# olegroshka/vae-channel-dynamics

Measured on AMD Instinct MI355X. Metric: images/sec SDXL-VAE train step @256x256 (tracking on), higher is better.
Workload: dtype f32

## Files before the change

### vae-channel-dynamics_amd/csrc/igemm.hip

```cpp
#include "bf16_frag.h"
#include <algorithm>
#include <stdlib.h>
#include <type_traits>

#include "launchers.h"

namespace {

struct LanePos {
  int lr, lh, trq, trp, trh;
};
__device__ __forceinline__ LanePos lane_pos(int lane) { return LanePos{lane & 31, lane >> 5, (lane & 15) >> 2, lane & 3, (lane >> 4) & 1}; }

struct F32 {
  typedef float elem;
  typedef f32x4 raw4;
  typedef f32x4 frag;
  typedef unsigned off_t;
  static constexpr int BK_ROWS = 32, BK_WGRAD = 32;
  static constexpr int KG = 8;
  static constexpr int PAD_K = 4, PAD_T = 4;
  static constexpr bool SETPRIO = true;
  static constexpr bool PAIR16 = false;
  static constexpr bool flag(int32_t) { return false; }

  static __device__ __forceinline__ raw4 load4(__amdgpu_buffer_rsrc_t rs, unsigned, bool ok, int row, int ld, int c) {
    return VAE_BUF_LOAD4(rs, oob_unless(ok, ((unsigned)row * (unsigned)ld + (unsigned)c) * 4u));
  }
  static __device__ __forceinline__ f32x4 to_f32(raw4 r, bool) { return r; }
  static __device__ __forceinline__ void put4(elem* d, f32x4 v) { *reinterpret_cast<f32x4*>(d) = v; }
  static __device__ __forceinline__ void put4_stored(elem* d, raw4, f32x4 v, bool) { put4(d, v); }
  static __device__ __forceinline__ frag frag_k(const elem* p) { return *reinterpret_cast<const f32x4*>(p); }
  static __device__ __forceinline__ frag frag_t(const elem* tile, int ld, int kg, LanePos l, int col0) {
    frag v;
#pragma unroll
    for (int j = 0; j < 4; ++j) v[j] = tile[(kg * 8 + l.lh * 4 + j) * ld + col0 + l.lr];
    return v;
  }
  template <int MI, int NI>
  static __device__ __forceinline__ void frags_tt(frag* a, frag* b, const elem* sA, int ldA, int colA, const elem* sB, int ldB, int colB, int kg, LanePos l) {
#pragma unroll
    for (int j = 0; j < 4; ++j) {
      const int k = kg * 8 + l.lh * 4 + j;
#pragma unroll
      for (int mi = 0; mi < MI; ++mi) a[mi][j] = sA[k * ldA + colA + mi * 32 + l.lr];
#pragma unroll
      for (int ni = 0; ni < NI; ++ni) b[ni][j] = sB[k * ldB + colB + ni * 32 + l.lr];
    }
  }
  template <int MI, int NI>
  static __device__ __forceinline__ void mma(f32x16 (&acc)[MI][NI], const frag* a, const frag* b) {
#pragma unroll
    for (int j = 0; j < 4; ++j)
#pragma unroll
      for (int mi = 0; mi < MI; ++mi)
#pragma unroll
        for (int ni = 0; ni < NI; ++ni) acc[mi][ni] = __builtin_amdgcn_mfma_f32_32x32x2f32(a[mi][j], b[ni][j], acc[mi][ni], 0, 0, 0);
  }
  static __device__ __forceinline__ off_t out_off(bool ok, int orow, int ldc, int col) {
    return ok ? ((unsigned)orow * (unsigned)ldc + (unsigned)col) * 4u : BUF_OOB;
  }
  static __device__ __forceinline__ bool inside(off_t o) { return o != BUF_OOB; }
  static __device__ __forceinline__ float load1(__amdgpu_buffer_rsrc_t rs, bool, off_t o) {
    return __builtin_bit_cast(float, __builtin_amdgcn_raw_buffer_load_b32(rs, o, 0, 0));
  }
  static __device__ __forceinline__ void store1(__amdgpu_buffer_rsrc_t rs, bool, off_t o, float v) {
    __builtin_amdgcn_raw_buffer_store_b32(__builtin_bit_cast(unsigned, v), rs, o, 0, 0);
  }
};

struct BF16 {
  typedef u16 elem;
  typedef uint4 raw4;
  typedef bf16x8 frag;
  typedef int off_t;
  static constexpr int BK_ROWS = 64, BK_WGRAD = 32;
  static constexpr int KG = 16;
  static constexpr int PAD_K = 8, PAD_T = 32;
  static constexpr bool SETPRIO = false;
  static constexpr bool PAIR16 = true;
  static __device__ __forceinline__ bool flag(int32_t v) { return v != 0; }

  static __device__ __forceinline__ raw4 load4(__amdgpu_buffer_rsrc_t rs, unsigned esize, bool ok, int row, int ld, int c) {
    return buf_load4_raw(rs, esize, neg_unless(ok, row * ld + c));
  }
  static __device__ __forceinline__ f32x4 to_f32(raw4 r, bool bf) { return raw4_to_f32(r, bf); }
  static __device__ __forceinline__ void put4(elem* d, f32x4 v) { *reinterpret_cast<uint2*>(d) = pack4(v); }
  static __device__ __forceinline__ void put4_stored(elem* d, raw4 r, f32x4 v, bool bf) {
    *reinterpret_cast<uint2*>(d) = bf ? uint2{r.x, r.y} : pack4(v);
  }
  static __device__ __forceinline__ frag frag_k(const elem* p) { return frag_direct(p); }
  static __device__ __forceinline__ frag frag_t(const elem* tile, int ld, int kg, LanePos l, int col0) {
    return frag_tr(tile + (kg * 16 + l.lh * 8 + l.trq) * ld + col0 + l.trh * 16 + l.trp * 4, ld);
  }
  template <int MI, int NI>
  static __device__ __forceinline__ void frags_tt(frag* a, frag* b, const elem* sA, int ldA, int colA, const elem* sB, int ldB, int colB, int kg, LanePos l) {
#pragma unroll
    for (int mi = 0; mi < MI; ++mi) a[mi] = frag_t(sA, ldA, kg, l, colA + mi * 32);
#pragma unroll
    for (int ni = 0; ni < NI; ++ni) b[ni] = frag_t(sB, ldB, kg, l, colB + ni * 32);
  }
  template <int MI, int NI>
  static __device__ __forceinline__ void mma(f32x16 (&acc)[MI][NI], const frag* a, const frag* b) {
#pragma unroll
    for (int mi = 0; mi < MI; ++mi)
#pragma unroll
      for (int ni = 0; ni < NI; ++ni) acc[mi][ni] = __builtin_amdgcn_mfma_f32_32x32x16_bf16(a[mi], b[ni], acc[mi][ni], 0, 0, 0);
  }
  static __device__ __forceinline__ off_t out_off(bool ok, int orow, int ldc, int col) { return ok ? orow * ldc + col : -1; }
  static __device__ __forceinline__ bool inside(off_t o) { return o >= 0; }
  static __device__ __forceinline__ float load1(__amdgpu_buffer_rsrc_t rs, bool bf, off_t o) { return buf_load1_elem(rs, bf, o); }
  static __device__ __forceinline__ void store1(__amdgpu_buffer_rsrc_t rs, bool bf, off_t o, float v) { buf_store1_elem(rs, bf, o, v); }

  static __device__ __forceinline__ bool pair16(const vae_igemm_args& p, bool cbf, bool rbf, const char* C) {
    return cbf && (p.N % 2 == 0) && (p.ldc % 2 == 0) && (p.res == nullptr || rbf) && p.track == nullptr && ((reinterpret_cast<uintptr_t>(C) & 3u) == 0);
  }
  template <int MI, int NI, class RowPixel>
  static __device__ __forceinline__ void store_pairs(const vae_igemm_args& p, const f32x16 (&acc)[MI][NI], int ni, __amdgpu_buffer_rsrc_t rsC,
                                                     __amdgpu_buffer_rsrc_t rsR, int col, bool colok, int m0, int trow0, int lh, bool s2c,
                                                     RowPixel row_pixel) {
    const bool odd = col & 1;
    const float b0 = (p.bias && colok) ? p.bias[col & ~1] : 0.f, b1 = (p.bias && colok) ? p.bias[col | 1] : 0.f;
#pragma unroll
    for (int mi = 0; mi < MI; ++mi) {
      unsigned o16[8], rr[8];
#pragma unroll
      for (int j = 0; j < 8; ++j) {
        const int r = 2 * j + (odd ? 1 : 0);
        const int row = trow0 + mi * 32 + (r & 3) + 8 * (r >> 2) + 4 * lh;
        int orow = row;
        if (s2c) {
          int b, y, x;
          row_pixel(row < p.M ? row : m0, b, y, x);
          orow = (b * p.g.Ho + y) * p.g.Wo + x;
        }
        o16[j] = (colok && row < p.M) ? (unsigned)(orow * p.ldc + (col & ~1)) * 2u : BUF_OOB;
        rr[j] = 0u;
      }
      if (p.res) {
#pragma unroll
        for (int j = 0; j < 8; ++j) rr[j] = __builtin_amdgcn_raw_buffer_load_b32(rsR, o16[j], 0, 0);
      }
#pragma unroll
      for (int j = 0; j < 8; ++j) {
        const float a0 = p.alpha * acc[mi][ni][2 * j], a1 = p.alpha * acc[mi][ni][2 * j + 1];
        const float recv = lane_xor1(odd ? a0 : a1);
        typedef __bf16 bf16x2_t __attribute__((ext_vector_type(2)));
        bf16x2_t h;
        h[0] = (__bf16)((odd ? recv : a0) + b0 + __builtin_bit_cast(float, rr[j] << 16));
        h[1] = (__bf16)((odd ? a1 : recv) + b1 + __builtin_bit_cast(float, rr[j] & 0xffff0000u));
        __builtin_amdgcn_raw_buffer_store_b32(__builtin_bit_cast(unsigned, h), rsC, o16[j], 0, 0);
      }
    }
  }
};

template <int MI, int NI>
__device__ __forceinline__ void zero_acc(f32x16 (&acc)[MI][NI]) {
#pragma unroll
  for (int mi = 0; mi < MI; ++mi)
#pragma unroll
    for (int ni = 0; ni < NI; ++ni)
#pragma unroll
      for (int r = 0; r < 16; ++r) acc[mi][ni][r] = 0.f;
}

template <class P, int BM, int BN, int WM, int WN, bool BKM, bool VEC, int XF>
__device__ __forceinline__ void rows_body(const vae_igemm_args& p) {
  typedef typename P::elem elem;
  constexpr int BK = P::BK_ROWS;
  constexpr int NT = 64 * WM * WN;
  constexpr int KQ = BK / 4;
  constexpr int RP = NT / KQ;
  constexpr int LDA = BK + P::PAD_K;
  constexpr int LDB = BKM ? (BN + P::PAD_T) : (BK + P::PAD_K);
  constexpr int SA = BM * LDA;
  constexpr int SB = BKM ? BK * LDB : BN * LDB;
  constexpr int STAGE = SA + SB;
  constexpr int SS = (XF != VAE_XF_NONE) ? 2 * SS_HALF * (4 / (int)sizeof(elem)) : 0;
  constexpr int TM = BM / WM, TN = BN / WN, MI = TM / 32, NI = TN / 32;
  constexpr int AR = BM / RP;
  constexpr int NQ = BN / 4, KR = NT / NQ;
  constexpr int BR = BKM ? (BK / KR) : (BN / RP);
  static_assert(AR >= 1 && BR >= 1 && TM % 32 == 0 && TN % 32 == 0 && (BK / P::KG == 2 || BK / P::KG == 4), "tile/wave layout");
  __shared__ __attribute__((aligned(16))) elem smem[2 * STAGE + SS];
  float* sS = reinterpret_cast<float*>(smem + 2 * STAGE);

  const int tid = threadIdx.x, lane = tid & 63, wave = tid >> 6;
  const int wm = wave / WN, wn = wave % WN;
  const LanePos lp = lane_pos(lane);
  const int lr = lp.lr, lh = lp.lh;
  const int tilesN = (p.N + BN - 1) / BN;
  const int tm = blockIdx.x / tilesN, tn = blockIdx.x % tilesN;
  const int m0 = tm * BM, n0 = tn * BN;
  const int z = blockIdx.z;
  const vae_conv_geom g = p.g;
  const SrcMap smap = make_srcmap(g);
  const bool abf = P::flag(p.a_bf16), cbf = P::flag(p.out_bf16), rbf = P::flag(p.res_bf16);
  const unsigned esA = abf ? 2u : 4u;
  const char* __restrict__ A = reinterpret_cast<const char*>(p.A) + (int64_t)z * p.sAb * esA;
  const float* __restrict__ W = p.W + (int64_t)z * p.sWb;
  const int hw = g.Ho * g.Wo;

  const bool s2c = (g.mode == VAE_MODE_DGRAD_S2);
  const int hh = g.Ho >> 1, wh = g.Wo >> 1;
  const int cls_rows = s2c ? p.M >> 2 : 1;
  const int cls = s2c ? m0 / cls_rows : 0;
  const int cpy = cls >> 1, cpx = cls & 1;
  const int nkw = s2c ? (cpx ? 1 : 2) : 3;
  const int ntaps = s2c ? (cpy ? 1 : 2) * nkw : g.taps;
  auto row_pixel = [&](int m, int& b, int& y, int& x) {
    if (s2c) {
      const int r = m - cls * cls_rows;
      b = r / (hh * wh);
      const int rem = r - b * (hh * wh);
      const int i = rem / wh;
      y = 2 * i + cpy;
      x = 2 * (rem - i * wh) + cpx;
    } else {
      b = m / hw;
      const int rem = m - b * hw;
      y = rem / g.Wo;
      x = rem - y * g.Wo;
    }
  };

  const int b_base = s2c ? (m0 - cls * cls_rows) / (hh * wh) : m0 / hw;
  const size_t img = (size_t)g.Hs * g.Ws * g.Cs;
  const size_t abytes = (size_t)(g.B - b_base) * img * esA, wbytes = (size_t)(BKM ? (int64_t)p.K * p.sk : (int64_t)p.N * p.sn) * 4u;
  const auto rsA = VAE_BUF_RSRC(A + (int64_t)b_base * img * esA, abytes < BUF_MAX ? abytes : BUF_MAX);
  const auto rsW = VAE_BUF_RSRC(W, wbytes < BUF_MAX ? wbytes : BUF_MAX);

  const int k4 = tid % KQ, r0 = tid / KQ;
  const int n4 = tid % NQ, kq = tid / NQ;
  int rb[AR], ry[AR], rx[AR];
#pragma unroll
  for (int i = 0; i < AR; ++i) {
    const int m = m0 + r0 + RP * i;
// ... 26 lines not shown
  int a_b[AR];
  int reg_c0 = 0;

  auto load_regs = [&](int s) {
    const int ord = s / kchunks;
    const int c0 = (s - ord * kchunks) * BK;
    reg_c0 = c0;
    int kh, kw;
    if (s2c) {
      const int a = ord / nkw;
      kh = cpy ? 1 : 2 * a;
      kw = cpx ? 1 : 2 * (ord - a * nkw);
    } else {
      kh = (g.taps == 9) ? ord / 3 : 0;
      kw = (g.taps == 9) ? ord - kh * 3 : 0;
    }
    const int tap = kh * 3 + kw;
    const int c = c0 + k4 * 4;
#pragma unroll
    for (int i = 0; i < AR; ++i) {
      int sy = 0, sx = 0;
      const bool ok = src_pixel(smap, ry[i], rx[i], kh, kw, sy, sx) && (rb[i] >= 0);
      if constexpr (VEC) ra[i] = P::load4(rsA, esA, ok && c < p.K, ((rb[i] - b_base) * g.Hs + sy) * g.Ws + sx, g.Cs, c);
      else ra[i] = load4s(p.A + (int64_t)z * p.sAb + (((int64_t)rb[i] * g.Hs + sy) * g.Ws + sx) * g.Cs + c, ok, c, p.K);
      a_b[i] = ok ? rb[i] : -1;
    }
    if (!BKM) {
#pragma unroll
      for (int i = 0; i < BR; ++i) {
        const int n = n0 + r0 + RP * i;
        if constexpr (VEC) rw[i] = VAE_BUF_LOAD4(rsW, oob_unless(n < p.N && c < p.K, ((unsigned)n * (unsigned)p.sn + (unsigned)tap * (unsigned)p.st + (unsigned)c) * 4u));
        else rw[i] = load4s(W + (int64_t)n * p.sn + (int64_t)tap * p.st + c, n < p.N, c, p.K);
      }
    } else {
#pragma unroll
      for (int i = 0; i < BR; ++i) {
        const int k = c0 + kq + KR * i;
        const int n = n0 + n4 * 4;
        if constexpr (VEC) rw[i] = VAE_BUF_LOAD4(rsW, oob_unless(k < p.K && n < p.N, ((unsigned)k * (unsigned)p.sk + (unsigned)tap * (unsigned)p.st + (unsigned)n) * 4u));
        else rw[i] = load4s(W + (int64_t)k * p.sk + (int64_t)tap * p.st + n, k < p.K, n, p.N);
      }
    }
  };
  auto store_lds = [&](elem* sA, elem* sB) {
    const int c = reg_c0 + k4 * 4;
#pragma unroll
    for (int i = 0; i < AR; ++i) {
      f32x4 v = P::to_f32(ra[i], abf);
      if (XF != VAE_XF_NONE) {
        const bool ok = (a_b[i] >= 0) && (c < p.K);
        const int o = ok ? (a_b[i] - b_lo) * p.K + c : 0;
        v = xform4_tab<XF>(v, sS + o, sS + SS_HALF + o, ok);
      }
      P::put4(&sA[(r0 + RP * i) * LDA + k4 * 4], v);
    }
#pragma unroll
    for (int i = 0; i < BR; ++i) {
      if (!BKM) P::put4(&sB[(r0 + RP * i) * LDB + k4 * 4], rw[i]);
      else P::put4(&sB[(kq + KR * i) * LDB + n4 * 4], rw[i]);
    }
  };
  typename P::frag fa[2][MI], fb[2][NI];
  auto fetch = [&](const elem* sA, const elem* sB, int kg, typename P::frag* a, typename P::frag* b) {
#pragma unroll
    for (int mi = 0; mi < MI; ++mi) a[mi] = P::frag_k(&sA[(wm * TM + mi * 32 + lr) * LDA + kg * P::KG + lh * (P::KG / 2)]);
#pragma unroll
    for (int ni = 0; ni < NI; ++ni) {
      if (!BKM) b[ni] = P::frag_k(&sB[(wn * TN + ni * 32 + lr) * LDB + kg * P::KG + lh * (P::KG / 2)]);
      else b[ni] = P::frag_t(sB, LDB, kg, lp, wn * TN + ni * 32);
    }
  };
  constexpr int NKG = BK / P::KG;
  auto compute = [&](const elem* sA, const elem* sB, int kg) {
    if (kg + 1 < NKG) fetch(sA, sB, kg + 1, fa[(kg + 1) & 1], fb[(kg + 1) & 1]);
    __builtin_amdgcn_sched_barrier(0);
    if (P::SETPRIO) __builtin_amdgcn_s_setprio(1);
    P::mma(acc, fa[kg & 1], fb[kg & 1]);
    if (P::SETPRIO) __builtin_amdgcn_s_setprio(0);
    __builtin_amdgcn_sched_barrier(0);
  };
  load_regs(0);
  __syncthreads();
  store_lds(smem, smem + SA);
  if (steps > 1) load_regs(1);
  __syncthreads();
  for (int s = 0; s < steps; ++s) {
    const elem* cA = smem + (s & 1) * STAGE;
    const elem* cB = cA + SA;
    fetch(cA, cB, 0, fa[0], fb[0]);
    compute(cA, cB, 0);
    if (NKG == 4) compute(cA, cB, 1);
    if (s + 1 < steps) {
      elem* nA = smem + ((s + 1) & 1) * STAGE;
      store_lds(nA, nA + SA);
      if (s + 2 < steps) load_regs(s + 2);
    }
    compute(cA, cB, NKG / 2);
    if (NKG == 4) compute(cA, cB, 3);
    __syncthreads();
  }

  const unsigned esC = cbf ? 2u : 4u, esR = rbf ? 2u : 4u;
  char* __restrict__ C = reinterpret_cast<char*>(p.C) + (int64_t)z * p.sCb * esC;
  const auto rsC = VAE_BUF_RSRC(C, (size_t)p.M * p.ldc * esC);
  const auto rsR = VAE_BUF_RSRC(p.res ? reinterpret_cast<const char*>(p.res) + (int64_t)z * p.sCb * esR : C, (size_t)p.M * p.ldc * (p.res ? esR : esC));
  float tsum[NI];
#pragma unroll
  for (int ni = 0; ni < NI; ++ni) tsum[ni] = 0.f;
  bool pair16 = false;
  if constexpr (P::PAIR16) pair16 = P::pair16(p, cbf, rbf, C);
#pragma unroll
  for (int ni = 0; ni < NI; ++ni) {
    const int col = n0 + wn * TN + ni * 32 + lr;
    const bool colok = col < p.N;
    const float bv = (p.bias && colok) ? p.bias[col] : 0.f;
    if constexpr (P::PAIR16) {
      if (pair16) {
        P::store_pairs(p, acc, ni, rsC, rsR, col, colok, m0, m0 + wm * TM, lh, s2c, row_pixel);
        continue;
      }
    }
#pragma unroll
    for (int mi = 0; mi < MI; ++mi) {
      typename P::off_t off[16];
      float rv[16];
#pragma unroll
      for (int r = 0; r < 16; ++r) {
        const int row = m0 + wm * TM + mi * 32 + (r & 3) + 8 * (r >> 2) + 4 * lh;
        int orow = row;
        if (s2c) {
          int b, y, x;
          row_pixel(row < p.M ? row : m0, b, y, x);
          orow = (b * g.Ho + y) * g.Wo + x;
        }
        off[r] = P::out_off(colok && row < p.M, orow, p.ldc, col);
        rv[r] = 0.f;
      }
      if (p.res) {
#pragma unroll
        for (int r = 0; r < 16; ++r) rv[r] = P::load1(rsR, rbf, off[r]);
      }
#pragma unroll
      for (int r = 0; r < 16; ++r) {
        const float v = p.alpha * acc[mi][ni][r] + bv + rv[r];
        P::store1(rsC, cbf, off[r], v);
        tsum[ni] += P::inside(off[r]) ? fabsf(v) : 0.f;
      }
    }
  }
  if (p.track && z == 0) {
    float* red = reinterpret_cast<float*>(smem);
#pragma unroll
    for (int ni = 0; ni < NI; ++ni) {
      const float s2 = tsum[ni] + __shfl_xor(tsum[ni], 32, 64);
      if (lh == 0) red[wm * BN + wn * TN + ni * 32 + lr] = s2;
    }
    __syncthreads();
    if (tid < BN) {
      float t = 0.f;
#pragma unroll
      for (int w = 0; w < WM; ++w) t += red[w * BN + tid];
      if (n0 + tid < p.N) p.track[(int64_t)tm * p.N + n0 + tid] = t;
    }
  }
}

template <class P, int BM, int BN, int WM, int WN, bool VEC, int XF>
__device__ __forceinline__ void wgrad_body(const vae_wgrad_args& p) {
  typedef typename P::elem elem;
  constexpr int BK = P::BK_WGRAD;
  constexpr int NT = 64 * WM * WN;
  constexpr int LDA = BM + P::PAD_T, LDB = BN + P::PAD_T;
  constexpr int SA = BK * LDA, SB = BK * LDB;
  constexpr int STAGE = SA + SB;
  constexpr int SS = (XF != VAE_XF_NONE) ? 2 * SS_HALF * (4 / (int)sizeof(elem)) : 0;
  constexpr int TM = BM / WM, TN = BN / WN, MI = TM / 32, NI = TN / 32;
  constexpr int AQ = BM / 4, AKR = NT / AQ, AI = BK / AKR;
  constexpr int BQ = BN / 4, BKR = NT / BQ, BI = BK / BKR;
  static_assert(AI >= 1 && BI >= 1 && TM % 32 == 0 && TN % 32 == 0 && (BK / P::KG == 2 || BK / P::KG == 4), "tile/wave layout");
  __shared__ __attribute__((aligned(16))) elem smem[2 * STAGE + SS];
  float* sS = reinterpret_cast<float*>(smem + 2 * STAGE);

  const int tid = threadIdx.x, lane = tid & 63, wave = tid >> 6;
  const int wm = wave / WN, wn = wave % WN;
  const LanePos lp = lane_pos(lane);
  const int lr = lp.lr, lh = lp.lh;
  const int tilesN = (p.N + BN - 1) / BN;
  const int tm = blockIdx.x / tilesN, tn = blockIdx.x % tilesN;
  const int m0 = tm * BM, n0 = tn * BN;
  const int tap = blockIdx.y / p.nsplit, split = blockIdx.y % p.nsplit;
  const int z = blockIdx.z;
  const vae_conv_geom g = p.g;
  const SrcMap smap = make_srcmap(g);
  const int kh = (g.taps == 9) ? tap / 3 : 0, kw = (g.taps == 9) ? tap - kh * 3 : 0;
  const bool ybf = P::flag(p.y_bf16), xbf = P::flag(p.x_bf16);
  const unsigned esY = ybf ? 2u : 4u, esX = xbf ? 2u : 4u;
  const char* __restrict__ dY = reinterpret_cast<const char*>(p.dY) + (int64_t)z * p.sYb * esY;
  const char* __restrict__ X = reinterpret_cast<const char*>(p.X) + (int64_t)z * p.sXb * esX;

  int chunk = (p.npix + p.nsplit - 1) / p.nsplit;
  chunk = ((chunk + 31) / 32) * 32;
  const int pbeg = split * chunk;
  const int pend = min(p.npix, pbeg + chunk);
  const int steps = (pend > pbeg) ? (pend - pbeg + BK - 1) / BK : 0;
  const int hw = g.Ho * g.Wo;
  const bool do_bias = (p.bias_partial != nullptr) && tn == 0 && tap == 0 && z == 0;

  const int b_lo = pbeg / hw;
  if (XF != VAE_XF_NONE && steps > 0) {
    const int nb = (pend - 1) / hw - b_lo + 1;
    const int ncol = min(BN, p.N - n0);
    const int nent = min(nb * BN, SS_HALF);
    for (int i = tid; i < nent; i += NT) {
      const int j = i / BN, c = i - j * BN;
      const bool ok = c < ncol;
      sS[i] = ok ? p.scale[(int64_t)(b_lo + j) * g.Cs + n0 + c] : 0.f;
      sS[SS_HALF + i] = ok ? p.shift[(int64_t)(b_lo + j) * g.Cs + n0 + c] : 0.f;
    }
  }

  f32x16 acc[MI][NI];
  zero_acc(acc);

  const size_t img = (size_t)g.Hs * g.Ws * g.Cs;
  const size_t ybytes = (size_t)(steps > 0 ? pend - pbeg : 0) * p.ldy * esY, xbytes = (size_t)(g.B - b_lo) * img * esX;
  const auto rsY = VAE_BUF_RSRC(dY + (int64_t)pbeg * p.ldy * esY, ybytes < BUF_MAX ? ybytes : BUF_MAX);
  const auto rsX = VAE_BUF_RSRC(X + (int64_t)b_lo * img * esX, xbytes < BUF_MAX ? xbytes : BUF_MAX);

  const int a4 = tid % AQ, akq = tid / AQ;
  const int b4 = tid % BQ, bkq = tid / BQ;
  typename P::raw4 ra[AI], rx[BI];
  int xb[BI];
  f32x4 bsum = {0.f, 0.f, 0.f, 0.f};

  auto load_regs = [&](int s) {
    const int pb = pbeg + s * BK;
#pragma unroll
    for (int i = 0; i < AI; ++i) {
      const int pix = pb + akq + AKR * i;
      const int c = m0 + a4 * 4;
      if constexpr (VEC) ra[i] = P::load4(rsY, esY, pix < pend && c < p.M, pix - pbeg, p.ldy, c);
      else ra[i] = load4s(p.dY + (int64_t)z * p.sYb + (int64_t)pix * p.ldy + c, pix < pend, c, p.M);
    }
#pragma unroll
    for (int i = 0; i < BI; ++i) {
      const int pix = pb + bkq + BKR * i;
      const int c = n0 + b4 * 4;
      const int b = pix / hw, rem = pix - b * hw;
      const int y = rem / g.Wo, x = rem - y * g.Wo;
      int sy = 0, sx = 0;
      const bool ok = src_pixel(smap, y, x, kh, kw, sy, sx) && (pix < pend);
      if constexpr (VEC) rx[i] = P::load4(rsX, esX, ok && c < p.N, ((b - b_lo) * g.Hs + sy) * g.Ws + sx, g.Cs, c);
      else rx[i] = load4s(p.X + (int64_t)z * p.sXb + (((int64_t)b * g.Hs + sy) * g.Ws + sx) * g.Cs + c, ok, c, p.N);
      xb[i] = ok ? b : -1;
    }
  };
  auto store_lds = [&](elem* sA, elem* sB) {
#pragma unroll
    for (int i = 0; i < AI; ++i) {
      const f32x4 v = P::to_f32(ra[i], ybf);
      P::put4_stored(&sA[(akq + AKR * i) * LDA + a4 * 4], ra[i], v, ybf);
      if (do_bias) bsum += v;
    }
#pragma unroll
    for (int i = 0; i < BI; ++i) {
      f32x4 v = P::to_f32(rx[i], xbf);
      if (XF != VAE_XF_NONE) {
        const bool ok = xb[i] >= 0;
        const int o = ok ? (xb[i] - b_lo) * BN + b4 * 4 : 0;
        v = xform4_tab<XF>(v, sS + o, sS + SS_HALF + o, ok);
      }
      P::put4(&sB[(bkq + BKR * i) * LDB + b4 * 4], v);
    }
  };
  typename P::frag fa[2][MI], fb[2][NI];
  auto fetch = [&](const elem* sA, const elem* sB, int kg, typename P::frag* a, typename P::frag* b) {
    P::template frags_tt<MI, NI>(a, b, sA, LDA, wm * TM, sB, LDB, wn * TN, kg, lp);
  };
  constexpr int NKG = BK / P::KG;
  auto compute = [&](const elem* sA, const elem* sB, int kg) {
    if (kg + 1 < NKG) fetch(sA, sB, kg + 1, fa[(kg + 1) & 1], fb[(kg + 1) & 1]);
    __builtin_amdgcn_sched_barrier(0);
    if (P::SETPRIO) __builtin_amdgcn_s_setprio(1);
    P::mma(acc, fa[kg & 1], fb[kg & 1]);
    if (P::SETPRIO) __builtin_amdgcn_s_setprio(0);
    __builtin_amdgcn_sched_barrier(0);
  };
  if (steps > 0) {
    load_regs(0);
    __syncthreads();
    store_lds(smem, smem + SA);
    if (steps > 1) load_regs(1);
    __syncthreads();
    for (int s = 0; s < steps; ++s) {
      const elem* cA = smem + (s & 1) * STAGE;
      const elem* cB = cA + SA;
      fetch(cA, cB, 0, fa[0], fb[0]);
      compute(cA, cB, 0);
      if (NKG == 4) compute(cA, cB, 1);
      if (s + 1 < steps) {
        elem* nA = smem + ((s + 1) & 1) * STAGE;
        store_lds(nA, nA + SA);
        if (s + 2 < steps) load_regs(s + 2);
      }
      compute(cA, cB, NKG / 2);
      if (NKG == 4) compute(cA, cB, 3);
      __syncthreads();
    }
  }

  const int64_t ld = (int64_t)g.taps * p.N;
  float* __restrict__ O = (p.nsplit == 1 ? p.out : p.partial + (int64_t)split * p.M * ld) + (int64_t)z * p.sOb;
#pragma unroll
  for (int ni = 0; ni < NI; ++ni) {
    const int col = n0 + wn * TN + ni * 32 + lr;
    if (col >= p.N) continue;
#pragma unroll
    for (int mi = 0; mi < MI; ++mi)
#pragma unroll
      for (int r = 0; r < 16; ++r) {
        const int row = m0 + wm * TM + mi * 32 + (r & 3) + 8 * (r >> 2) + 4 * lh;
        if (row < p.M) O[(int64_t)row * ld + (int64_t)tap * p.N + col] = p.alpha * acc[mi][ni][r];
      }
  }
  if (do_bias) {
    f32x4* red = reinterpret_cast<f32x4*>(smem);
    red[akq * AQ + a4] = bsum;
    __syncthreads();
    if (tid < AQ) {
      f32x4 t = {0.f, 0.f, 0.f, 0.f};
      for (int r = 0; r < AKR; ++r) t += red[r * AQ + tid];
#pragma unroll
      for (int e = 0; e < 4; ++e) {
        const int m = m0 + tid * 4 + e;
        if (m < p.M) p.bias_partial[(int64_t)split * p.M + m] = t[e];
      }
    }
  }
}

template <int BM, int BN, int WM, int WN, bool BKM, bool VEC, int XF>
__global__ __launch_bounds__(64 * WM * WN) void igemm_rows_kernel(vae_igemm_args p) { rows_body<F32, BM, BN, WM, WN, BKM, VEC, XF>(p); }
template <int BM, int BN, int WM, int WN, bool VEC, int XF>
__global__ __launch_bounds__(64 * WM * WN) void wgrad_kernel(vae_wgrad_args p) { wgrad_body<F32, BM, BN, WM, WN, VEC, XF>(p); }
template <int BM, int BN, int WM, int WN, bool BKM, int XF>
__global__ __launch_bounds__(64 * WM * WN) void igemm_rows_bf16_kernel(vae_igemm_args p) { rows_body<BF16, BM, BN, WM, WN, BKM, true, XF>(p); }
template <int BM, int BN, int WM, int WN, int XF>
__global__ __launch_bounds__(64 * WM * WN) void wgrad_bf16_kernel(vae_wgrad_args p) { wgrad_body<BF16, BM, BN, WM, WN, true, XF>(p); }

__device__ __forceinline__ void small_column_sums(const float* __restrict__ partial2, int nsplit, int n2, float* __restrict__ out2, int blk) {
  const int i = blk * 256 + (int)threadIdx.x;
  if (i >= n2) return;
  const float* p = partial2 + i;
  float s = 0.f;
  int k = 0;
  for (; k + 16 <= nsplit; k += 16) {
    float v[16];
#pragma unroll
    for (int j = 0; j < 16; ++j) v[j] = p[(int64_t)(k + j) * n2];
#pragma unroll
    for (int j = 0; j < 16; ++j) s += v[j];
  }
  for (; k < nsplit; ++k) s += p[(int64_t)k * n2];
  out2[i] = s;
}

template <int KP>
__global__ __launch_bounds__(256) void reduce_splits_kernel(const float* __restrict__ partial, int nsplit, int64_t n, float* __restrict__ out,
                                                            int main_blocks, const float* __restrict__ partial2, int n2, float* __restrict__ out2) {
  constexpr int COLS = 256 / KP;
  __shared__ f32x4 red[KP > 1 ? 256 : 1];
  if ((int)blockIdx.x >= main_blocks) {
    small_column_sums(partial2, nsplit, n2, out2, (int)blockIdx.x - main_blocks);
    return;
  }
  const int col = threadIdx.x % COLS, kp = threadIdx.x / COLS;
  const int64_t n4 = n >> 2;
  const int per = (nsplit + KP - 1) / KP;
  const int k0 = kp * per, k1 = min(nsplit, k0 + per);
  auto column = [&](int64_t i) {
    f32x4 s = {0.f, 0.f, 0.f, 0.f};
    const f32x4* p = reinterpret_cast<const f32x4*>(partial) + i;
    int k = k0;
    for (; k + 8 <= k1; k += 8) {
      f32x4 v[8];
#pragma unroll
      for (int j = 0; j < 8; ++j) v[j] = p[(int64_t)(k + j) * n4];
      s += ((v[0] + v[1]) + (v[2] + v[3])) + ((v[4] + v[5]) + (v[6] + v[7]));
    }
    for (; k < k1; ++k) s += p[(int64_t)k * n4];
    return s;
  };
  if (KP == 1) {
    for (int64_t i = (int64_t)blockIdx.x * 256 + threadIdx.x; i < n4; i += (int64_t)main_blocks * 256) reinterpret_cast<f32x4*>(out)[i] = column(i);
    return;
  }
  const int64_t i = (int64_t)blockIdx.x * COLS + col;
// ... 101 lines not shown
    f32x4 o[9];
    if constexpr (NPOS == 16) {
      f32x4 h[3][4];
#pragma unroll
      for (int j = 0; j < 4; ++j) {
        const float cj = (j == 1 || j == 2) ? 0.5f : 1.f;
        const f32x4 r0 = acc[0 * 4 + j] * cj, r1 = acc[1 * 4 + j] * (0.5f * cj), r2 = acc[2 * 4 + j] * (0.5f * cj), r3 = acc[3 * 4 + j] * cj;
        h[0][j] = (r0 + r1) + r2;
        h[1][j] = r1 - r2;
        h[2][j] = (r1 + r2) - r3;
      }
#pragma unroll
      for (int a = 0; a < 3; ++a) {
        o[a * 3 + 0] = (h[a][0] + h[a][1]) + h[a][2];
        o[a * 3 + 1] = h[a][1] - h[a][2];
        o[a * 3 + 2] = (h[a][1] + h[a][2]) - h[a][3];
      }
    } else {
      f32x4 h[3][3];
#pragma unroll
      for (int j = 0; j < 3; ++j) {
        h[0][j] = acc[0 * 3 + j] + acc[1 * 3 + j];
        h[1][j] = acc[1 * 3 + j];
        h[2][j] = acc[1 * 3 + j] - acc[2 * 3 + j];
      }
#pragma unroll
      for (int a = 0; a < 3; ++a) {
        o[a * 3 + 0] = h[a][0] + h[a][1];
        o[a * 3 + 1] = h[a][1];
        o[a * 3 + 2] = h[a][1] - h[a][2];
      }
    }
#pragma unroll
    for (int t = 0; t < 9; ++t)
#pragma unroll
      for (int e = 0; e < 4; ++e) sT[t][4 * cq + e][cl] = o[t][e];
  }
  __syncthreads();
  for (int idx = tid; idx < 9 * TCO * TCI; idx += 256) {
    const int c = idx % TCI, r = idx / TCI;
    const int t = r % 9, ml = r / 9;
    dW[((int64_t)(m0 + ml) * 9 + t) * N + c0 + c] = sT[t][ml][c];
  }
}

using std::false_type;
using std::true_type;

template <bool BF, int BM, int BN, int WM, int WN>
int launch_rows_tile(const vae_igemm_args& a, bool bkm, bool vec, hipStream_t st) {
  const dim3 grid((unsigned)(((a.M + BM - 1) / BM) * ((a.N + BN - 1) / BN)), 1, (unsigned)a.batch), block(64 * WM * WN);
  auto go = [&](auto bkm_c, auto vec_c) {
    constexpr bool BKM = decltype(bkm_c)::value, VEC = decltype(vec_c)::value;
    auto launch = [&](auto xf) {
      if constexpr (BF) hipLaunchKernelGGL((igemm_rows_bf16_kernel<BM, BN, WM, WN, BKM, decltype(xf)::value>), grid, block, 0, st, a);
      else hipLaunchKernelGGL((igemm_rows_kernel<BM, BN, WM, WN, BKM, VEC, decltype(xf)::value>), grid, block, 0, st, a);
    };
    if constexpr (BKM) {
      if (a.xf != VAE_XF_NONE) { vae_set_error("igemm_rows: xf unsupported with n-contiguous weights"); return VAE_EINVAL; }
      launch(int_c<VAE_XF_NONE>{});
    } else if (!dispatch_xf(a.xf, launch)) {
      vae_set_error("igemm_rows: bad xf %d", a.xf);
      return VAE_EINVAL;
    }
    return 0;
  };
  if (BF || vec) return bkm ? go(true_type{}, true_type{}) : go(false_type{}, true_type{});
  if constexpr (!BF) return bkm ? go(true_type{}, false_type{}) : go(false_type{}, false_type{});
  return 0;
}
template <bool BF>
int launch_rows(const vae_igemm_args& a, bool bkm, bool vec, hipStream_t st) {
  return (a.N <= 32) ? launch_rows_tile<BF, 128, 32, 4, 1>(a, bkm, vec, st) : launch_rows_tile<BF, 128, 128, 4, 2>(a, bkm, vec, st);
}

template <bool BF, int BM, int BN, int WM, int WN>
int launch_wgrad_tile(const vae_wgrad_args& a, bool vec, hipStream_t st) {
  const dim3 grid((unsigned)(((a.M + BM - 1) / BM) * ((a.N + BN - 1) / BN)), (unsigned)(a.g.taps * a.nsplit), (unsigned)a.batch), block(64 * WM * WN);
  auto go = [&](auto vec_c) {
    auto launch = [&](auto xf) {
      if constexpr (BF) hipLaunchKernelGGL((wgrad_bf16_kernel<BM, BN, WM, WN, decltype(xf)::value>), grid, block, 0, st, a);
      else hipLaunchKernelGGL((wgrad_kernel<BM, BN, WM, WN, decltype(vec_c)::value, decltype(xf)::value>), grid, block, 0, st, a);
    };
    if (dispatch_xf(a.xf, launch)) return 0;
    vae_set_error("wgrad: bad xf %d", a.xf);
    return VAE_EINVAL;
  };
  if (BF || vec) return go(true_type{});
  if constexpr (!BF) return go(false_type{});
  return 0;
}
template <bool BF>
int launch_wgrad(const vae_wgrad_args& a, bool vec, hipStream_t st) {
  if (a.M <= 32) return launch_wgrad_tile<BF, 32, 128, 1, 4>(a, vec, st);
  if (a.N <= 32) return launch_wgrad_tile<BF, 128, 32, 4, 1>(a, vec, st);
  return launch_wgrad_tile<BF, 128, 128, 4, 2>(a, vec, st);
}

}

int launch_rows_f32(const vae_igemm_args& a, bool bkm, bool vec, hipStream_t st) { return launch_rows<false>(a, bkm, vec, st); }
int launch_rows_bf16(const vae_igemm_args& a, bool bkm, hipStream_t st) { return launch_rows<true>(a, bkm, true, st); }
int launch_wgrad_f32(const vae_wgrad_args& a, bool vec, hipStream_t st) { return launch_wgrad<false>(a, vec, st); }
int launch_wgrad_bf16(const vae_wgrad_args& a, hipStream_t st) { return launch_wgrad<true>(a, true, st); }

static int reduce_splits_impl(const float* partial, int32_t nsplit, int64_t n, float* out, const float* partial2, int32_t n2, float* out2,
                              hipStream_t st) {
  const int extra = partial2 ? (n2 + 255) / 256 : 0;
  if (n % 4 == 0 && aligned16(partial) && aligned16(out)) {
    const int64_t n4 = n / 4;
    if (nsplit >= 32) {
      const int64_t blocks = (n4 + 63) / 64;
      VAE_CHECK(blocks + extra < (1ll << 31), "reduce_splits: too many elements");
      hipLaunchKernelGGL(reduce_splits_kernel<4>, dim3((unsigned)(blocks + extra)), dim3(256), 0, st, partial, nsplit, n, out, (int)blocks, partial2, n2, out2);
    } else {
      const int64_t blocks = std::min<int64_t>((n4 + 255) / 256, 8192);
      hipLaunchKernelGGL(reduce_splits_kernel<1>, dim3((unsigned)(blocks + extra)), dim3(256), 0, st, partial, nsplit, n, out, (int)blocks, partial2, n2, out2);
    }
  } else {
    int blocks = (int)((n + 255) / 256);
    if (blocks > 4096) blocks = 4096;
    hipLaunchKernelGGL(reduce_splits_scalar_kernel, dim3(blocks), dim3(256), 0, st, partial, nsplit, n, out);
    if (partial2) hipLaunchKernelGGL(reduce_splits_scalar_kernel, dim3(extra), dim3(256), 0, st, partial2, nsplit, (int64_t)n2, out2);
  }
  return 0;
}
extern "C" int vae_reduce_splits(const float* partial, int32_t nsplit, int64_t n, float* out, void* stream) {
  VAE_CHECK(partial && out && nsplit > 0 && n > 0, "reduce_splits: bad args");
  if (int rc = reduce_splits_impl(partial, nsplit, n, out, nullptr, 0, nullptr, (hipStream_t)stream)) return rc;
  VAE_LAUNCH_CHECK("reduce_splits");
  return VAE_OK;
}
extern "C" int vae_reduce_splits2(const float* partial, int32_t nsplit, int64_t n, float* out, const float* partial2, int32_t n2, float* out2,
                                  void* stream) {
  VAE_CHECK(partial && out && partial2 && out2 && nsplit > 0 && n > 0 && n2 > 0, "reduce_splits2: bad args");
  if (int rc = reduce_splits_impl(partial, nsplit, n, out, partial2, n2, out2, (hipStream_t)stream)) return rc;
  VAE_LAUNCH_CHECK("reduce_splits2");
// ... 30 lines not shown
```

Baseline: 107.1.

## Emulate f32 GEMM with split-bf16 three-plane MFMA for 8-wave tiles

Adds an F32X3 path that splits each f32 operand into three bf16 planes (hi, mid, lo) when staging to LDS, then accumulates six bf16 32x32x16 MFMA products per k-group instead of using the 32x32x2 f32 MFMA. It applies to vectorized 8-wave rows and wgrad kernels (128x128 tiles), with BK reduced to 16 and LDS moved to dynamic allocation because the three planes need more space. This trades the slow native f32 MFMA rate for higher bf16 throughput, at the cost of extra conversion ALU work, triple LDS footprint, and slightly different rounding from true f32.

```diff
diff --git a/vae-channel-dynamics_amd/csrc/igemm.hip b/vae-channel-dynamics_amd/csrc/igemm.hip
--- a/vae-channel-dynamics_amd/csrc/igemm.hip
+++ b/vae-channel-dynamics_amd/csrc/igemm.hip
@@ -22,23 +22,26 @@
   static constexpr int PAD_K = 4, PAD_T = 4;
   static constexpr bool SETPRIO = true;
   static constexpr bool PAIR16 = false;
+  static constexpr int PLANES = 1;
+  static constexpr bool LDS_DYNAMIC = false;
   static constexpr bool flag(int32_t) { return false; }
 
   static __device__ __forceinline__ raw4 load4(__amdgpu_buffer_rsrc_t rs, unsigned, bool ok, int row, int ld, int c) {
     return VAE_BUF_LOAD4(rs, oob_unless(ok, ((unsigned)row * (unsigned)ld + (unsigned)c) * 4u));
   }
   static __device__ __forceinline__ f32x4 to_f32(raw4 r, bool) { return r; }
-  static __device__ __forceinline__ void put4(elem* d, f32x4 v) { *reinterpret_cast<f32x4*>(d) = v; }
-  static __device__ __forceinline__ void put4_stored(elem* d, raw4, f32x4 v, bool) { put4(d, v); }
-  static __device__ __forceinline__ frag frag_k(const elem* p) { return *reinterpret_cast<const f32x4*>(p); }
-  static __device__ __forceinline__ frag frag_t(const elem* tile, int ld, int kg, LanePos l, int col0) {
+  static __device__ __forceinline__ void put4(elem* d, f32x4 v, int) { *reinterpret_cast<f32x4*>(d) = v; }
+  static __device__ __forceinline__ void put4_stored(elem* d, raw4, f32x4 v, bool, int) { put4(d, v, 0); }
+  static __device__ __forceinline__ frag frag_k(const elem* p, int) { return *reinterpret_cast<const f32x4*>(p); }
+  static __device__ __forceinline__ frag frag_t(const elem* tile, int ld, int kg, LanePos l, int col0, int) {
     frag v;
 #pragma unroll
     for (int j = 0; j < 4; ++j) v[j] = tile[(kg * 8 + l.lh * 4 + j) * ld + col0 + l.lr];
     return v;
   }
   template <int MI, int NI>
-  static __device__ __forceinline__ void frags_tt(frag* a, frag* b, const elem* sA, int ldA, int colA, const elem* sB, int ldB, int colB, int kg, LanePos l) {
+  static __device__ __forceinline__ void frags_tt(frag* a, frag* b, const elem* sA, int ldA, int colA, const elem* sB, int ldB, int colB, int kg, LanePos l,
+                                                  int, int) {
 #pragma unroll
     for (int j = 0; j < 4; ++j) {
       const int k = kg * 8 + l.lh * 4 + j;
@@ -79,26 +82,29 @@
   static constexpr int PAD_K = 8, PAD_T = 32;
   static constexpr bool SETPRIO = false;
   static constexpr bool PAIR16 = true;
+  static constexpr int PLANES = 1;
+  static constexpr bool LDS_DYNAMIC = false;
   static __device__ __forceinline__ bool flag(int32_t v) { return v != 0; }
 
   static __device__ __forceinline__ raw4 load4(__amdgpu_buffer_rsrc_t rs, unsigned esize, bool ok, int row, int ld, int c) {
     return buf_load4_raw(rs, esize, neg_unless(ok, row * ld + c));
   }
   static __device__ __forceinline__ f32x4 to_f32(raw4 r, bool bf) { return raw4_to_f32(r, bf); }
-  static __device__ __forceinline__ void put4(elem* d, f32x4 v) { *reinterpret_cast<uint2*>(d) = pack4(v); }
-  static __device__ __forceinline__ void put4_stored(elem* d, raw4 r, f32x4 v, bool bf) {
+  static __device__ __forceinline__ void put4(elem* d, f32x4 v, int) { *reinterpret_cast<uint2*>(d) = pack4(v); }
+  static __device__ __forceinline__ void put4_stored(elem* d, raw4 r, f32x4 v, bool bf, int) {
     *reinterpret_cast<uint2*>(d) = bf ? uint2{r.x, r.y} : pack4(v);
   }
-  static __device__ __forceinline__ frag frag_k(const elem* p) { return frag_direct(p); }
-  static __device__ __forceinline__ frag frag_t(const elem* tile, int ld, int kg, LanePos l, int col0) {
+  static __device__ __forceinline__ frag frag_k(const elem* p, int) { return frag_direct(p); }
+  static __device__ __forceinline__ frag frag_t(const elem* tile, int ld, int kg, LanePos l, int col0, int) {
     return frag_tr(tile + (kg * 16 + l.lh * 8 + l.trq) * ld + col0 + l.trh * 16 + l.trp * 4, ld);
   }
   template <int MI, int NI>
-  static __device__ __forceinline__ void frags_tt(frag* a, frag* b, const elem* sA, int ldA, int colA, const elem* sB, int ldB, int colB, int kg, LanePos l) {
-#pragma unroll
-    for (int mi = 0; mi < MI; ++mi) a[mi] = frag_t(sA, ldA, kg, l, colA + mi * 32);
-#pragma unroll
-    for (int ni = 0; ni < NI; ++ni) b[ni] = frag_t(sB, ldB, kg, l, colB + ni * 32);
+  static __device__ __forceinline__ void frags_tt(frag* a, frag* b, const elem* sA, int ldA, int colA, const elem* sB, int ldB, int colB, int kg, LanePos l,
+                                                  int, int) {
+#pragma unroll
+    for (int mi = 0; mi < MI; ++mi) a[mi] = frag_t(sA, ldA, kg, l, colA + mi * 32, 0);
+#pragma unroll
+    for (int ni = 0; ni < NI; ++ni) b[ni] = frag_t(sB, ldB, kg, l, colB + ni * 32, 0);
   }
   template <int MI, int NI>
   static __device__ __forceinline__ void mma(f32x16 (&acc)[MI][NI], const frag* a, const frag* b) {
@@ -155,6 +161,82 @@
   }
 };
 
+#ifndef VAE_FLAT_X3
+#define VAE_FLAT_X3 1
+#endif
+struct F32X3 : F32 {
+  typedef u16 elem;
+  struct frag { bf16x8 p[3]; };
+  static constexpr int BK_ROWS = 16, BK_WGRAD = 16;
+  static constexpr int KG = 16;
+  static constexpr int PAD_K = 8, PAD_T = 32;
+  static constexpr bool SETPRIO = false;
+  static constexpr int PLANES = 3;
+  static constexpr bool LDS_DYNAMIC = true;
+
+  static __device__ __forceinline__ void put4(elem* d, f32x4 v, int ps) {
+    const uint2 hi = pack4(v);
+    const f32x4 h = unpack4(hi);
+    f32x4 r;
+#pragma unroll
+    for (int e = 0; e < 4; ++e) r[e] = v[e] - h[e];
+    const uint2 mid = pack4(r);
+    const f32x4 m = unpack4(mid);
+#pragma unroll
+    for (int e = 0; e < 4; ++e) r[e] = r[e] - m[e];
+    *reinterpret_cast<uint2*>(d) = hi;
+    *reinterpret_cast<uint2*>(d + ps) = mid;
+    *reinterpret_cast<uint2*>(d + 2 * ps) = pack4(r);
+  }
+  static __device__ __forceinline__ void put4_stored(elem* d, raw4, f32x4 v, bool, int ps) { put4(d, v, ps); }
+  static __device__ __forceinline__ frag frag_k(const elem* p, int ps) {
+    frag f;
+#pragma unroll
+    for (int q = 0; q < 3; ++q) f.p[q] = BF16::frag_k(p + q * ps, 0);
+    return f;
+  }
+  static __device__ __forceinline__ frag frag_t(const elem* tile, int ld, int kg, LanePos l, int col0, int ps) {
+    frag f;
+#pragma unroll
+    for (int q = 0; q < 3; ++q) f.p[q] = BF16::frag_t(tile + q * ps, ld, kg, l, col0, 0);
+    return f;
+  }
+  template <int MI, int NI>
+  static __device__ __forceinline__ void frags_tt(frag* a, frag* b, const elem* sA, int ldA, int colA, const elem* sB, int ldB, int colB, int kg, LanePos l,
+                                                  int psA, int psB) {
+#pragma unroll
+    for (int mi = 0; mi < MI; ++mi) a[mi] = frag_t(sA, ldA, kg, l, colA + mi * 32, psA);
+#pragma unroll
+    for (int ni = 0; ni < NI; ++ni) b[ni] = frag_t(sB, ldB, kg, l, colB + ni * 32, psB);
+  }
+  template <int MI, int NI>
+  static __device__ __forceinline__ void mma(f32x16 (&acc)[MI][NI], const frag* a, const frag* b) {
+    constexpr int PA[6] = {0, 2, 1, 0, 1, 0}, PB[6] = {2, 0, 1, 1, 0, 0};
+#pragma unroll
+    for (int t = 0; t < 6; ++t)
+#pragma unroll
+      for (int mi = 0; mi < MI; ++mi)
+#pragma unroll
+        for (int ni = 0; ni < NI; ++ni)
+          acc[mi][ni] = __builtin_amdgcn_mfma_f32_32x32x16_bf16(a[mi].p[PA[t]], b[ni].p[PB[t]], acc[mi][ni], 0, 0, 0);
+  }
+};
+
+template <bool VEC, int WAVES>
+using F32For = std::conditional_t<VEC && WAVES == 8 && (VAE_FLAT_X3 != 0), F32X3, F32>;
+
+template <class P, int BM, int BN, bool BKM, int XF>
+constexpr int rows_lds_elems() {
+  constexpr int BK = P::BK_ROWS;
+  return 2 * P::PLANES * (BM * (BK + P::PAD_K) + (BKM ? BK * (BN + P::PAD_T) : BN * (BK + P::PAD_K))) +
+         ((XF != VAE_XF_NONE) ? 2 * SS_HALF * (4 / (int)sizeof(typename P::elem)) : 0);
+}
+template <class P, int BM, int BN, int XF>
+constexpr int wgrad_lds_elems() {
+  return 2 * P::PLANES * P::BK_WGRAD * (BM + P::PAD_T + BN + P::PAD_T) + ((XF != VAE_XF_NONE) ? 2 * SS_HALF * (4 / (int)sizeof(typename P::elem)) : 0);
+}
+extern __shared__ __attribute__((aligned(16))) unsigned char lds_dynamic[];
+
 template <int MI, int NI>
 __device__ __forceinline__ void zero_acc(f32x16 (&acc)[MI][NI]) {
 #pragma unroll
@@ -176,14 +258,17 @@
   constexpr int LDB = BKM ? (BN + P::PAD_T) : (BK + P::PAD_K);
   constexpr int SA = BM * LDA;
   constexpr int SB = BKM ? BK * LDB : BN * LDB;
-  constexpr int STAGE = SA + SB;
+  constexpr int PL = P::PLANES;
+  constexpr int STAGE = PL * (SA + SB);
   constexpr int SS = (XF != VAE_XF_NONE) ? 2 * SS_HALF * (4 / (int)sizeof(elem)) : 0;
   constexpr int TM = BM / WM, TN = BN / WN, MI = TM / 32, NI = TN / 32;
   constexpr int AR = BM / RP;
   constexpr int NQ = BN / 4, KR = NT / NQ;
   constexpr int BR = BKM ? (BK / KR) : (BN / RP);
-  static_assert(AR >= 1 && BR >= 1 && TM % 32 == 0 && TN % 32 == 0 && (BK / P::KG == 2 || BK / P::KG == 4), "tile/wave layout");
-  __shared__ __attribute__((aligned(16))) elem smem[2 * STAGE + SS];
+  static_assert(AR >= 1 && BR >= 1 && TM % 32 == 0 && TN % 32 == 0 && (BK / P::KG == 1 || BK / P::KG == 2 || BK / P::KG == 4), "tile/wave layout");
+  static_assert(2 * STAGE + SS == rows_lds_elems<P, BM, BN, BKM, XF>(), "the launcher reserves what the body lays out");
+  __shared__ __attribute__((aligned(16))) elem smem_static[P::LDS_DYNAMIC ? 1 : 2 * STAGE + SS];
+  elem* const smem = P::LDS_DYNAMIC ? reinterpret_cast<elem*>(lds_dynamic) : smem_static;
   float* sS = reinterpret_cast<float*>(smem + 2 * STAGE);
 
   const int tid = threadIdx.x, lane = tid & 63, wave = tid >> 6;
@@ -316,22 +401,22 @@
         const int o = ok ? (a_b[i] - b_lo) * p.K + c : 0;
         v = xform4_tab<XF>(v, sS + o, sS + SS_HALF + o, ok);
       }
-      P::put4(&sA[(r0 + RP * i) * LDA + k4 * 4], v);
+      P::put4(&sA[(r0 + RP * i) * LDA + k4 * 4], v, SA);
     }
 #pragma unroll
     for (int i = 0; i < BR; ++i) {
-      if (!BKM) P::put4(&sB[(r0 + RP * i) * LDB + k4 * 4], rw[i]);
-      else P::put4(&sB[(kq + KR * i) * LDB + n4 * 4], rw[i]);
+      if (!BKM) P::put4(&sB[(r0 + RP * i) * LDB + k4 * 4], rw[i], SB);
+      else P::put4(&sB[(kq + KR * i) * LDB + n4 * 4], rw[i], SB);
     }
   };
   typename P::frag fa[2][MI], fb[2][NI];
   auto fetch = [&](const elem* sA, const elem* sB, int kg, typename P::frag* a, typename P::frag* b) {
 #pragma unroll
-    for (int mi = 0; mi < MI; ++mi) a[mi] = P::frag_k(&sA[(wm * TM + mi * 32 + lr) * LDA + kg * P::KG + lh * (P::KG / 2)]);
+    for (int mi = 0; mi < MI; ++mi) a[mi] = P::frag_k(&sA[(wm * TM + mi * 32 + lr) * LDA + kg * P::KG + lh * (P::KG / 2)], SA);
 #pragma unroll
     for (int ni = 0; ni < NI; ++ni) {
-      if (!BKM) b[ni] = P::frag_k(&sB[(wn * TN + ni * 32 + lr) * LDB + kg * P::KG + lh * (P::KG / 2)]);
-      else b[ni] = P::frag_t(sB, LDB, kg, lp, wn * TN + ni * 32);
+      if (!BKM) b[ni] = P::frag_k(&sB[(wn * TN + ni * 32 + lr) * LDB + kg * P::KG + lh * (P::KG / 2)], SB);
+      else b[ni] = P::frag_t(sB, LDB, kg, lp, wn * TN + ni * 32, SB);
     }
   };
   constexpr int NKG = BK / P::KG;
@@ -345,18 +430,18 @@
   };
   load_regs(0);
   __syncthreads();
-  store_lds(smem, smem + SA);
+  store_lds(smem, smem + PL * SA);
   if (steps > 1) load_regs(1);
   __syncthreads();
   for (int s = 0; s < steps; ++s) {
     const elem* cA = smem + (s & 1) * STAGE;
-    const elem* cB = cA + SA;
+    const elem* cB = cA + PL * SA;
     fetch(cA, cB, 0, fa[0], fb[0]);
-    compute(cA, cB, 0);
+    if (NKG > 1) compute(cA, cB, 0);
     if (NKG == 4) compute(cA, cB, 1);
     if (s + 1 < steps) {
       elem* nA = smem + ((s + 1) & 1) * STAGE;
-      store_lds(nA, nA + SA);
+      store_lds(nA, nA + PL * SA);
       if (s + 2 < steps) load_regs(s + 2);
     }
     compute(cA, cB, NKG / 2);
@@ -436,13 +521,16 @@
   constexpr int NT = 64 * WM * WN;
   constexpr int LDA = BM + P::PAD_T, LDB = BN + P::PAD_T;
   constexpr int SA = BK * LDA, SB = BK * LDB;
-  constexpr int STAGE = SA + SB;
+  constexpr int PL = P::PLANES;
+  constexpr int STAGE = PL * (SA + SB);
   constexpr int SS = (XF != VAE_XF_NONE) ? 2 * SS_HALF * (4 / (int)sizeof(elem)) : 0;
   constexpr int TM = BM / WM, TN = BN / WN, MI = TM / 32, NI = TN / 32;
   constexpr int AQ = BM / 4, AKR = NT / AQ, AI = BK / AKR;
   constexpr int BQ = BN / 4, BKR = NT / BQ, BI = BK / BKR;
-  static_assert(AI >= 1 && BI >= 1 && TM % 32 == 0 && TN % 32 == 0 && (BK / P::KG == 2 || BK / P::KG == 4), "tile/wave layout");
-  __shared__ __attribute__((aligned(16))) elem smem[2 * STAGE + SS];
+  static_assert(AI >= 1 && BI >= 1 && TM % 32 == 0 && TN % 32 == 0 && (BK / P::KG == 1 || BK / P::KG == 2 || BK / P::KG == 4), "tile/wave layout");
+  static_assert(2 * STAGE + SS == wgrad_lds_elems<P, BM, BN, XF>(), "the launcher reserves what the body lays out");
+  __shared__ __attribute__((aligned(16))) elem smem_static[P::LDS_DYNAMIC ? 1 : 2 * STAGE + SS];
+  elem* const smem = P::LDS_DYNAMIC ? reinterpret_cast<elem*>(lds_dynamic) : smem_static;
   float* sS = reinterpret_cast<float*>(smem + 2 * STAGE);
 
   const int tid = threadIdx.x, lane = tid & 63, wave = tid >> 6;
@@ -523,7 +611,7 @@
 #pragma unroll
     for (int i = 0; i < AI; ++i) {
       const f32x4 v = P::to_f32(ra[i], ybf);
-      P::put4_stored(&sA[(akq + AKR * i) * LDA + a4 * 4], ra[i], v, ybf);
+      P::put4_stored(&sA[(akq + AKR * i) * LDA + a4 * 4], ra[i], v, ybf, SA);
       if (do_bias) bsum += v;
     }
 #pragma unroll
@@ -534,12 +622,12 @@
         const int o = ok ? (xb[i] - b_lo) * BN + b4 * 4 : 0;
         v = xform4_tab<XF>(v, sS + o, sS + SS_HALF + o, ok);
       }
-      P::put4(&sB[(bkq + BKR * i) * LDB + b4 * 4], v);
+      P::put4(&sB[(bkq + BKR * i) * LDB + b4 * 4], v, SB);
     }
   };
   typename P::frag fa[2][MI], fb[2][NI];
   auto fetch = [&](const elem* sA, const elem* sB, int kg, typename P::frag* a, typename P::frag* b) {
-    P::template frags_tt<MI, NI>(a, b, sA, LDA, wm * TM, sB, LDB, wn * TN, kg, lp);
+    P::template frags_tt<MI, NI>(a, b, sA, LDA, wm * TM, sB, LDB, wn * TN, kg, lp, SA, SB);
   };
   constexpr int NKG = BK / P::KG;
   auto compute = [&](const elem* sA, const elem* sB, int kg) {
@@ -553,18 +641,18 @@
   if (steps > 0) {
     load_regs(0);
     __syncthreads();
-    store_lds(smem, smem + SA);
+    store_lds(smem, smem + PL * SA);
     if (steps > 1) load_regs(1);
     __syncthreads();
     for (int s = 0; s < steps; ++s) {
       const elem* cA = smem + (s & 1) * STAGE;
-      const elem* cB = cA + SA;
+      const elem* cB = cA + PL * SA;
       fetch(cA, cB, 0, fa[0], fb[0]);
-      compute(cA, cB, 0);
+      if (NKG > 1) compute(cA, cB, 0);
       if (NKG == 4) compute(cA, cB, 1);
       if (s + 1 < steps) {
         elem* nA = smem + ((s + 1) & 1) * STAGE;
-        store_lds(nA, nA + SA);
+        store_lds(nA, nA + PL * SA);
         if (s + 2 < steps) load_regs(s + 2);
       }
       compute(cA, cB, NKG / 2);
@@ -604,9 +692,9 @@
 }
 
 template <int BM, int BN, int WM, int WN, bool BKM, bool VEC, int XF>
-__global__ __launch_bounds__(64 * WM * WN) void igemm_rows_kernel(vae_igemm_args p) { rows_body<F32, BM, BN, WM, WN, BKM, VEC, XF>(p); }
+__global__ __launch_bounds__(64 * WM * WN) void igemm_rows_kernel(vae_igemm_args p) { rows_body<F32For<VEC, WM * WN>, BM, BN, WM, WN, BKM, VEC, XF>(p); }
 template <int BM, int BN, int WM, int WN, bool VEC, int XF>
-__global__ __launch_bounds__(64 * WM * WN) void wgrad_kernel(vae_wgrad_args p) { wgrad_body<F32, BM, BN, WM, WN, VEC, XF>(p); }
+__global__ __launch_bounds__(64 * WM * WN) void wgrad_kernel(vae_wgrad_args p) { wgrad_body<F32For<VEC, WM * WN>, BM, BN, WM, WN, VEC, XF>(p); }
 template <int BM, int BN, int WM, int WN, bool BKM, int XF>
 __global__ __launch_bounds__(64 * WM * WN) void igemm_rows_bf16_kernel(vae_igemm_args p) { rows_body<BF16, BM, BN, WM, WN, BKM, true, XF>(p); }
 template <int BM, int BN, int WM, int WN, int XF>
@@ -814,9 +902,18 @@
   const dim3 grid((unsigned)(((a.M + BM - 1) / BM) * ((a.N + BN - 1) / BN)), 1, (unsigned)a.batch), block(64 * WM * WN);
   auto go = [&](auto bkm_c, auto vec_c) {
     constexpr bool BKM = decltype(bkm_c)::value, VEC = decltype(vec_c)::value;
+    int rc = 0;
     auto launch = [&](auto xf) {
-      if constexpr (BF) hipLaunchKernelGGL((igemm_rows_bf16_kernel<BM, BN, WM, WN, BKM, decltype(xf)::value>), grid, block, 0, st, a);
-      else hipLaunchKernelGGL((igemm_rows_kernel<BM, BN, WM, WN, BKM, VEC, decltype(xf)::value>), grid, block, 0, st, a);
+      constexpr int XF = decltype(xf)::value;
+      if constexpr (BF) {
+        hipLaunchKernelGGL((igemm_rows_bf16_kernel<BM, BN, WM, WN, BKM, XF>), grid, block, 0, st, a);
+      } else if constexpr (F32For<VEC, WM * WN>::LDS_DYNAMIC) {
+        constexpr int LDS = rows_lds_elems<F32For<VEC, WM * WN>, BM, BN, BKM, XF>() * (int)sizeof(typename F32For<VEC, WM * WN>::elem);
+        if (rc == 0) rc = [&]() -> int { VAE_RESERVE_LDS((igemm_rows_kernel<BM, BN, WM, WN, BKM, VEC, XF>), LDS, "igemm_rows"); return 0; }();
+        if (rc == 0) hipLaunchKernelGGL((igemm_rows_kernel<BM, BN, WM, WN, BKM, VEC, XF>), grid, block, LDS, st, a);
+      } else {
+        hipLaunchKernelGGL((igemm_rows_kernel<BM, BN, WM, WN, BKM, VEC, XF>), grid, block, 0, st, a);
+      }
     };
     if constexpr (BKM) {
       if (a.xf != VAE_XF_NONE) { vae_set_error("igemm_rows: xf unsupported with n-contiguous weights"); return VAE_EINVAL; }
@@ -825,7 +922,7 @@
       vae_set_error("igemm_rows: bad xf %d", a.xf);
       return VAE_EINVAL;
     }
-    return 0;
+    return rc;
   };
   if (BF || vec) return bkm ? go(true_type{}, true_type{}) : go(false_type{}, true_type{});
   if constexpr (!BF) return bkm ? go(true_type{}, false_type{}) : go(false_type{}, false_type{});
@@ -840,11 +937,21 @@
 int launch_wgrad_tile(const vae_wgrad_args& a, bool vec, hipStream_t st) {
   const dim3 grid((unsigned)(((a.M + BM - 1) / BM) * ((a.N + BN - 1) / BN)), (unsigned)(a.g.taps * a.nsplit), (unsigned)a.batch), block(64 * WM * WN);
   auto go = [&](auto vec_c) {
+    int rc = 0;
     auto launch = [&](auto xf) {
-      if constexpr (BF) hipLaunchKernelGGL((wgrad_bf16_kernel<BM, BN, WM, WN, decltype(xf)::value>), grid, block, 0, st, a);
-      else hipLaunchKernelGGL((wgrad_kernel<BM, BN, WM, WN, decltype(vec_c)::value, decltype(xf)::value>), grid, block, 0, st, a);
+      constexpr bool VEC = decltype(vec_c)::value;
+      constexpr int XF = decltype(xf)::value;
+      if constexpr (BF) {
+        hipLaunchKernelGGL((wgrad_bf16_kernel<BM, BN, WM, WN, XF>), grid, block, 0, st, a);
+      } else if constexpr (F32For<VEC, WM * WN>::LDS_DYNAMIC) {
+        constexpr int LDS = wgrad_lds_elems<F32For<VEC, WM * WN>, BM, BN, XF>() * (int)sizeof(typename F32For<VEC, WM * WN>::elem);
+        if (rc == 0) rc = [&]() -> int { VAE_RESERVE_LDS((wgrad_kernel<BM, BN, WM, WN, VEC, XF>), LDS, "wgrad"); return 0; }();
+        if (rc == 0) hipLaunchKernelGGL((wgrad_kernel<BM, BN, WM, WN, VEC, XF>), grid, block, LDS, st, a);
+      } else {
+        hipLaunchKernelGGL((wgrad_kernel<BM, BN, WM, WN, VEC, XF>), grid, block, 0, st, a);
+      }
     };
-    if (dispatch_xf(a.xf, launch)) return 0;
+    if (dispatch_xf(a.xf, launch)) return rc;
     vae_set_error("wgrad: bad xf %d", a.xf);
     return VAE_EINVAL;
   };
```

After: 108.7, median of 6. 1.4% higher.
